# pierregab/VUB_Image_denoising

Measured on AMD Instinct MI355X. Metric: images/sec (256x256x3) RDUNet diffusion train step, higher is better.
Workload: dtype bf16; 1 GPU; RDUNet_T(base_filters=32) diffusion train step, fwd+Charbonnier+bwd+clip+AdamW; global_batch=16, per_gpu_batch=16, parallelism=dp1, optimizer_step=every step, launcher=single process

## Files before the change

vub_image_denoising_amd/csrc/pack.hip:

```cpp
#include "rdn_pointwise.h"

namespace {

__global__ void interp_kernel(const float* __restrict__ clean, const float* __restrict__ noisy,
                              const float* __restrict__ tn, int batch, int64_t per, float* __restrict__ x) {
  const int64_t n4 = per / 4;
  const int64_t total = (int64_t)batch * n4;
  for (int64_t i = (int64_t)blockIdx.x * blockDim.x + threadIdx.x; i < total; i += (int64_t)gridDim.x * blockDim.x) {
    const int b = (int)(i / n4);
    const float a = tn[b];
    const f32x4 c = ((const f32x4*)clean)[i], n = ((const f32x4*)noisy)[i];
    ((f32x4*)x)[i] = a * n + (1.f - a) * c;
  }
}

template <typename T>
__global__ void pack_input_kernel(const float* __restrict__ x, int N, int C, int H, int W, const float* __restrict__ t,
                                  int64_t t_sb, int64_t t_sh, int64_t t_sw, int has_t, T* __restrict__ out, int cpad) {
  const int64_t HW = (int64_t)H * W, P = (int64_t)N * HW;
  for (int64_t p = (int64_t)blockIdx.x * blockDim.x + threadIdx.x; p < P; p += (int64_t)gridDim.x * blockDim.x) {
    const int64_t n = p / HW, r = p - n * HW;
    const int y = (int)(r / W), xx = (int)(r - (int64_t)y * W);
    T* o = out + p * cpad;
    for (int c = 0; c < cpad; ++c) {
      float v = 0.f;
      if (c < C) v = x[(n * C + c) * HW + r];
      else if (c == C && has_t) v = t[n * t_sb + y * t_sh + xx * t_sw];
      o[c] = from_f32<T>(v);
    }
  }
}

__device__ __forceinline__ float pack_value(int mode, const float* __restrict__ w, int d0, int d1, int kh, int kw,
                                            int pad0, int pad1, int kc, int ck, int r, int k) {
  const int taps = kh * kw;
  if (mode == RDN_PACK_CONV_FWD) {
    int tap, b;
    if (ck > 0) { const int ch = k / kc, rem = k - ch * kc; tap = rem / ck; b = ch * ck + (rem - tap * ck); }
    else { tap = k / pad1; b = k - tap * pad1; }
    const int a = r;
    if (a < d0 && b < d1 && tap < taps) return w[((int64_t)a * d1 + b) * taps + tap];
  } else if (mode == RDN_PACK_CONV_DGRAD) {
    int tp, a;
    if (ck > 0) { const int ch = k / kc, rem = k - ch * kc; tp = rem / ck; a = ch * ck + (rem - tp * ck); }
    else { tp = k / pad0; a = k - tp * pad0; }
    const int b = r;
    if (a < d0 && b < d1 && tp < taps) {
      const int ky = kh - 1 - tp / kw, kx = kw - 1 - tp % kw;
      return w[((int64_t)a * d1 + b) * taps + ky * kw + kx];
    }
  } else {
    const int tap = r / d1, b = r - tap * d1, a = k;
    if (tap < taps && a < d0) return w[((int64_t)a * d1 + b) * taps + tap];
  }
  return 0.f;
}

static inline int chunk_sk(int dtype) { return dtype == RDN_BF16 ? 64 : 32; }
static inline int chunk_kc(int ck, int dtype) {
  const int sk = chunk_sk(dtype);
  return ck > 0 ? (9 * ck + sk - 1) / sk * sk : 0;
}

template <typename T>
__global__ void pack_weights_kernel(int mode, const float* __restrict__ w, int d0, int d1, int kh, int kw, int pad0,
                                    int pad1, T* __restrict__ out, int rows_pad, int kp, int ck, int kc) {
  const int64_t total = (int64_t)rows_pad * kp;
  for (int64_t i = (int64_t)blockIdx.x * blockDim.x + threadIdx.x; i < total; i += (int64_t)gridDim.x * blockDim.x) {
    const int r = (int)(i / kp), k = (int)(i - (int64_t)r * kp);
    out[i] = from_f32<T>(pack_value(mode, w, d0, d1, kh, kw, pad0, pad1, kc, ck, r, k));
  }
}

template <typename T>
__global__ __launch_bounds__(256) void pack_weights_batched_kernel(const rdn_pack_item* __restrict__ items, int sk) {
  constexpr int VEC = TypeInfo<T>::VEC;
  const rdn_pack_item it = items[blockIdx.y];
  const int kc = it.ck > 0 ? (9 * it.ck + sk - 1) / sk * sk : 0;
  const int units = it.rows_pad * (it.kp / VEC);
  T* __restrict__ out = (T*)it.out;
  for (int u = blockIdx.x * 256 + threadIdx.x; u < units; u += gridDim.x * 256) {
    const int e = u * VEC, r = e / it.kp, k0 = e - r * it.kp;
    float v[VEC];
#pragma unroll
    for (int q = 0; q < VEC; ++q)
      v[q] = pack_value(it.mode, it.w, it.d0, it.d1, it.kh, it.kw, it.pad0, it.pad1, kc, it.ck, r, k0 + q);
    *(u32x4*)(out + e) = Unit16<T>::pack(v);
  }
}

__global__ void sampling_combine_kernel(float* __restrict__ x, const float* __restrict__ f1, const float* __restrict__ f2,
                                        const float* __restrict__ y, int64_t n, float c1, float a, float c2, float ap) {
#pragma clang fp contract(off)
  for (int64_t i = (int64_t)blockIdx.x * blockDim.x + threadIdx.x; i < n; i += (int64_t)gridDim.x * blockDim.x) {
    const float xt = c1 * f1[i] + a * y[i];
    const float xp = c2 * f2[i] + ap * y[i];
    x[i] = (x[i] - xt) + xp;
  }
}

template <typename T>
__global__ void nchw_to_nhwc_kernel(const float* __restrict__ s, int N, int C, int H, int W, T* __restrict__ d,
                                    int64_t ps, int c0, int64_t pl, int acc) {
  const int64_t HW = (int64_t)H * W, total = (int64_t)N * C * HW;
  for (int64_t i = (int64_t)blockIdx.x * blockDim.x + threadIdx.x; i < total; i += (int64_t)gridDim.x * blockDim.x) {
    const int64_t p = i / C;
    const int c = (int)(i - p * C);
    const int64_t n = p / HW, r = p - n * HW;
    T* const o = d + p * ps + rdn_coff(c0 + c, ps, pl);
    const float v = s[(n * C + c) * HW + r];
    *o = from_f32<T>(acc ? to_f32(*o) + v : v);
  }
}

template <typename T>
__global__ void nhwc_to_nchw_kernel(const T* __restrict__ s, int64_t ps, int c0, int64_t pl, int N, int C, int H, int W,
                                    float* __restrict__ d, int acc) {
  const int64_t HW = (int64_t)H * W, total = (int64_t)N * C * HW;
  for (int64_t i = (int64_t)blockIdx.x * blockDim.x + threadIdx.x; i < total; i += (int64_t)gridDim.x * blockDim.x) {
    const int64_t r = i % HW, nc = i / HW;
    const int c = (int)(nc % C);
    const int64_t n = nc / C;
    const float v = to_f32(s[(n * HW + r) * ps + rdn_coff(c0 + c, ps, pl)]);
    d[i] = acc ? d[i] + v : v;
  }
}

template <typename T>
__global__ void zero_slice_kernel(T* __restrict__ d, int64_t pixels, int64_t ps, int c0, int cols) {
  const int64_t total = pixels * cols;
  for (int64_t i = (int64_t)blockIdx.x * blockDim.x + threadIdx.x; i < total; i += (int64_t)gridDim.x * blockDim.x) {
    const int64_t p = i / cols;
    const int c = (int)(i - p * cols);
    d[p * ps + c0 + c] = from_f32<T>(0.f);
  }
}

}

extern "C" int rdn_interp(const float* clean, const float* noisy, const float* tnorm, int32_t batch, int64_t per,
                          float* x, void* stream) {
  if (!clean || !noisy || !tnorm || !x || per % 4 || ((uintptr_t)clean | (uintptr_t)noisy | (uintptr_t)x) & 15) {
    rdn_set_error("rdn_interp: bad arguments"); return RDN_E_ARG;
  }
  interp_kernel<<<grid_for(batch * per / 4, 256), 256, 0, RDN_STREAM>>>(clean, noisy, tnorm, batch, per, x);
  return rdn_check_launch("rdn_interp");
}

extern "C" int rdn_pack_input(int32_t dtype, const float* x, int32_t n, int32_t c, int32_t h, int32_t w, const float* t,
                              int64_t t_sb, int64_t t_sh, int64_t t_sw, int32_t has_t, void* out, int32_t cpad,
                              void* stream) {
  if (!x || !out || (has_t && !t) || cpad < c + (has_t ? 1 : 0)) { rdn_set_error("rdn_pack_input: bad arguments"); return RDN_E_ARG; }
  const int64_t P = (int64_t)n * h * w;
  RDN_LAUNCH_T(dtype, pack_input_kernel<T><<<grid_for(P, 256), 256, 0, RDN_STREAM>>>(x, n, c, h, w, t, t_sb, t_sh, t_sw, has_t,
                                                                                   (T*)out, cpad));
  return rdn_check_launch("rdn_pack_input");
}

extern "C" int rdn_pack_weights_batched(const rdn_pack_item* items, int32_t n, int32_t dtype, void* stream) {
  if (!items || n <= 0 || n > 65535) { rdn_set_error("rdn_pack_weights_batched: bad arguments"); return RDN_E_ARG; }
  dim3 grid(96, n);
  RDN_LAUNCH_T(dtype, pack_weights_batched_kernel<T><<<grid, 256, 0, RDN_STREAM>>>(items, chunk_sk(dtype)));
  return rdn_check_launch("rdn_pack_weights_batched");
}

extern "C" int rdn_pack_weights(int32_t mode, int32_t dtype, const float* w, int32_t d0, int32_t d1, int32_t kh,
                                int32_t kw, int32_t pad0, int32_t pad1, void* out, int32_t rows_pad, int32_t kp,
                                int32_t ck, void* stream) {
  if (!w || !out || mode < 0 || mode > 2 || kp % 64 || rows_pad % 128) { rdn_set_error("rdn_pack_weights: bad arguments"); return RDN_E_ARG; }
  const int taps = kh * kw;
  const int kc = chunk_kc(ck, dtype);
  if (ck > 0) {
    const int kside = mode == RDN_PACK_CONV_FWD ? pad1 : pad0;
    if (taps != 9 || mode == RDN_PACK_GEMM_T || kside % ck || (kside / ck) * kc > kp) {
      rdn_set_error("rdn_pack_weights: chunked pack needs a 3x3 conv mode and kp >= %d", (kside / ck) * kc);
      return RDN_E_SHAPE;
    }
  } else if ((mode == RDN_PACK_CONV_FWD && (pad1 < d1 || rows_pad < d0 || taps * pad1 > kp)) ||
      (mode == RDN_PACK_CONV_DGRAD && (pad0 < d0 || rows_pad < d1 || taps * pad0 > kp)) ||
      (mode == RDN_PACK_GEMM_T && (pad0 < d0 || pad0 > kp || rows_pad < taps * d1))) {
    rdn_set_error("rdn_pack_weights: shape (mode=%d d0=%d d1=%d pad0=%d pad1=%d rows=%d kp=%d)", mode, d0, d1, pad0, pad1,
                  rows_pad, kp);
    return RDN_E_SHAPE;
  }
  const int64_t total = (int64_t)rows_pad * kp;
  RDN_LAUNCH_T(dtype, pack_weights_kernel<T><<<grid_for(total, 256), 256, 0, RDN_STREAM>>>(mode, w, d0, d1, kh, kw, pad0, pad1,
                                                                                         (T*)out, rows_pad, kp, ck, kc));
  return rdn_check_launch("rdn_pack_weights");
}

extern "C" int rdn_sampling_combine(float* x, const float* f1, const float* f2, const float* y, int64_t count, float c1,
                                    float a, float c2, float ap, void* stream) {
  if (!x || !f1 || !f2 || !y || count <= 0) { rdn_set_error("rdn_sampling_combine: bad arguments"); return RDN_E_ARG; }
  sampling_combine_kernel<<<grid_for(count, 256 * 4), 256, 0, RDN_STREAM>>>(x, f1, f2, y, count, c1, a, c2, ap);
  return rdn_check_launch("rdn_sampling_combine");
}

extern "C" int rdn_nchw_to_nhwc(int32_t dtype, const float* src, int32_t n, int32_t c, int32_t h, int32_t w, void* dst,
                                int64_t dst_ps, int32_t dst_c0, int64_t dst_pl, int32_t accumulate, void* stream) {
  if (!src || !dst || dst_ps <= 0) { rdn_set_error("rdn_nchw_to_nhwc: null / bad stride"); return RDN_E_ARG; }
  const int64_t total = (int64_t)n * c * h * w;
  RDN_LAUNCH_T(dtype, nchw_to_nhwc_kernel<T><<<grid_for(total, 256 * 4), 256, 0, RDN_STREAM>>>(src, n, c, h, w, (T*)dst, dst_ps,
                                                                                             dst_c0, dst_pl, accumulate));
  return rdn_check_launch("rdn_nchw_to_nhwc");
}

extern "C" int rdn_nhwc_to_nchw(int32_t dtype, const void* src, int64_t src_ps, int32_t src_c0, int64_t src_pl, int32_t n,
                                int32_t c, int32_t h, int32_t w, float* dst, int32_t accumulate, void* stream) {
  if (!src || !dst || src_ps <= 0) { rdn_set_error("rdn_nhwc_to_nchw: null / bad stride"); return RDN_E_ARG; }
  const int64_t total = (int64_t)n * c * h * w;
  RDN_LAUNCH_T(dtype, nhwc_to_nchw_kernel<T><<<grid_for(total, 256 * 4), 256, 0, RDN_STREAM>>>((const T*)src, src_ps, src_c0, src_pl,
                                                                                             n, c, h, w, dst, accumulate));
  return rdn_check_launch("rdn_nhwc_to_nchw");
}

extern "C" int rdn_zero_slice(int32_t dtype, void* dst, int64_t pixels, int64_t ps, int32_t c0, int32_t cols, void* stream) {
  if (!dst || pixels < 0 || cols < 0) { rdn_set_error("rdn_zero_slice: bad arguments"); return RDN_E_ARG; }
  if (pixels == 0 || cols == 0) return RDN_OK;
  RDN_LAUNCH_T(dtype, zero_slice_kernel<T><<<grid_for(pixels * cols, 256 * 4), 256, 0, RDN_STREAM>>>((T*)dst, pixels, ps, c0, cols));
  return rdn_check_launch("rdn_zero_slice");
}
```

Measured before the change: 1875 images/s.

## Restructure batched weight pack into LDS-staged tiles with balanced persistent scheduling

```diff
diff --git a/vub_image_denoising_amd/csrc/pack.hip b/vub_image_denoising_amd/csrc/pack.hip
--- a/vub_image_denoising_amd/csrc/pack.hip
+++ b/vub_image_denoising_amd/csrc/pack.hip
@@ -1,3 +1,5 @@
+#include "rdn_device.h"
+#include "rdn_launch.h"
 #include "rdn_pointwise.h"
 
 namespace {
@@ -72,20 +74,224 @@
   }
 }
 
-template <typename T>
-__global__ __launch_bounds__(256) void pack_weights_batched_kernel(const rdn_pack_item* __restrict__ items, int sk) {
+constexpr int PK_XT = 64;
+constexpr int PK_RT = 8;
+constexpr int PK_NT = 256;
+constexpr int PK_U = 5;
+constexpr int PK_SLOTS = PK_NT * PK_U;
+constexpr int PK_LDS = PK_XT * 82;
+constexpr int PK_IPT = 2;
+constexpr int PK_MAXN = PK_NT * PK_IPT;
+
+__device__ __forceinline__ int div_small(int i, float inv) { return (int)(((float)i + 0.5f) * inv); }
+
+struct PackGeom {
+  int taps, kc, seg_w, chunk_k, pitch, rt, row_span, taps_out, nch, nxt, ntiles;
+  bool fwd, gemm, gather;
+};
+
+template <typename T>
+__device__ __forceinline__ PackGeom pack_geom(const rdn_pack_item& it, int sk) {
   constexpr int VEC = TypeInfo<T>::VEC;
-  const rdn_pack_item it = items[blockIdx.y];
-  const int kc = it.ck > 0 ? (9 * it.ck + sk - 1) / sk * sk : 0;
-  const int units = it.rows_pad * (it.kp / VEC);
+  PackGeom g;
+  g.taps = it.kh * it.kw;
+  g.kc = it.ck > 0 ? (9 * it.ck + sk - 1) / sk * sk : 0;
+  g.fwd = it.mode == RDN_PACK_CONV_FWD, g.gemm = it.mode == RDN_PACK_GEMM_T;
+  g.seg_w = g.gemm ? it.kp : it.ck > 0 ? it.ck : g.fwd ? it.pad1 : it.pad0;
+  g.chunk_k = it.ck > 0 ? g.kc : it.kp;
+  const int taps1 = max(g.taps, 1);
+  g.rt = g.fwd ? min(PK_RT, PK_SLOTS / ((PK_XT * taps1 + 6) / 4)) : min(32, (4 * (PK_SLOTS / PK_XT) - 3) / taps1);
+  g.pitch = g.fwd ? PK_XT * taps1 + 1 : (g.rt * taps1 + 6) / 8 * 8 + 1;
+  g.gather = g.taps <= 0 || g.seg_w <= 0 || g.seg_w % VEC || it.d0 <= 0 || it.d1 <= 0 || g.chunk_k <= 0 ||
+             it.rows_pad >= (1 << 20) ||
+             (it.ck > 0 && g.taps * g.seg_w > g.chunk_k) || g.rt <= 0 || (g.fwd ? g.rt : PK_XT) * g.pitch > PK_LDS;
+  if (g.gather) {
+    g.ntiles = (it.rows_pad * (it.kp / VEC) + PK_NT - 1) / PK_NT;
+    return g;
+  }
+  g.row_span = g.gemm ? it.d1 : it.rows_pad;
+  g.taps_out = g.gemm ? (it.rows_pad + it.d1 - 1) / it.d1 : g.taps;
+  g.nch = (it.kp + g.chunk_k - 1) / g.chunk_k, g.nxt = (g.seg_w + PK_XT - 1) / PK_XT;
+  g.ntiles = (g.row_span + g.rt - 1) / g.rt * g.nch * g.nxt;
+  return g;
+}
+
+template <typename T>
+__device__ void pack_gather_box(const rdn_pack_item& it, const PackGeom& g, int tile) {
+  constexpr int VEC = TypeInfo<T>::VEC;
+  const int u = tile * PK_NT + threadIdx.x;
+  if (u >= it.rows_pad * (it.kp / VEC)) return;
+  const int e = u * VEC, r = e / it.kp, k0 = e - r * it.kp;
+  float v[VEC];
+#pragma unroll
+  for (int q = 0; q < VEC; ++q)
+    v[q] = pack_value(it.mode, it.w, it.d0, it.d1, it.kh, it.kw, it.pad0, it.pad1, g.kc, it.ck, r, k0 + q);
+  *(u32x4*)((T*)it.out + e) = Unit16<T>::pack(v);
+}
+
+struct PackBox {
+  int xt, ch, r0, xw, xbase, rows_l;
+};
+__device__ __forceinline__ PackBox pack_box_at(const PackGeom& g, int tile) {
+  PackBox b;
+  b.xt = tile % g.nxt, b.ch = (tile / g.nxt) % g.nch, b.r0 = (tile / (g.nxt * g.nch)) * g.rt;
+  b.xw = min(PK_XT, g.seg_w - b.xt * PK_XT);
+  b.xbase = (g.gemm ? 0 : b.ch * g.seg_w) + b.xt * PK_XT;
+  b.rows_l = min(g.rt, g.row_span - b.r0);
+  return b;
+}
+
+struct PackRegs {
+  f32x4 f[PK_U];
+  int l0[PK_U], lo[PK_U], hi[PK_U];
+};
+
+__device__ __forceinline__ void pack_box_fetch(const rdn_pack_item& it, const PackGeom& g, int tile, PackRegs& R) {
+  const PackBox b = pack_box_at(g, tile);
+  const int taps = g.taps, total = it.d0 * it.d1 * taps;
+  const int wal = (int)(((uintptr_t)it.w >> 2) & 3);
+  const float* __restrict__ wa = it.w - wal;
+  const int a_base = g.fwd ? b.r0 : b.xbase, b_base = g.fwd ? b.xbase : b.r0;
+  const int nruns = max(min(g.fwd ? b.rows_l : b.xw, it.d0 - a_base), 0);
+  const int n = max(min(g.fwd ? b.xw : b.rows_l, it.d1 - b_base), 0) * taps;
+  const int nv = (n + 6) / 4;
+  const float inv_nv = 1.f / (float)nv;
+#pragma unroll
+  for (int s = 0; s < PK_U; ++s) {
+    const int i = threadIdx.x + s * PK_NT;
+    R.lo[s] = R.hi[s] = R.l0[s] = 0;
+    if (n == 0 || i >= nruns * nv) continue;
+    const int j = div_small(i, inv_nv), v = i - j * nv;
+    const int g0 = wal + ((a_base + j) * it.d1 + b_base) * taps;
+    const int e0 = (g0 & ~3) + 4 * v;
+    R.l0[s] = j * g.pitch + e0 - g0;
+    R.lo[s] = max(g0 - e0, 0), R.hi[s] = min(g0 + n - e0, 4);
+    if (e0 >= wal && e0 + 4 <= wal + total) R.f[s] = *(const f32x4*)(wa + e0);
+    else {
+#pragma unroll
+      for (int q = 0; q < 4; ++q)
+        if (q >= R.lo[s] && q < R.hi[s]) R.f[s][q] = wa[e0 + q];
+    }
+  }
+}
+
+__device__ __forceinline__ void pack_box_stage(const PackRegs& R, float* __restrict__ lds) {
+#pragma unroll
+  for (int s = 0; s < PK_U; ++s) {
+    if (R.lo[s] == 0 && R.hi[s] == 4) {
+#pragma unroll
+      for (int q = 0; q < 4; ++q) lds[R.l0[s] + q] = R.f[s][q];
+    } else {
+#pragma unroll
+      for (int q = 0; q < 4; ++q)
+        if (q >= R.lo[s] && q < R.hi[s]) lds[R.l0[s] + q] = R.f[s][q];
+    }
+  }
+}
+
+template <typename T>
+__device__ __forceinline__ void pack_box_emit(const rdn_pack_item& it, const PackGeom& g, int tile,
+                                              const float* __restrict__ lds) {
+  constexpr int VEC = TypeInfo<T>::VEC, XG = PK_XT / VEC;
+  const PackBox b = pack_box_at(g, tile);
+  const bool fwd = g.fwd, gemm = g.gemm;
+  const int taps = g.taps, seg_w = g.seg_w;
   T* __restrict__ out = (T*)it.out;
-  for (int u = blockIdx.x * 256 + threadIdx.x; u < units; u += gridDim.x * 256) {
-    const int e = u * VEC, r = e / it.kp, k0 = e - r * it.kp;
+  const int sr = fwd ? g.pitch : taps, sx = fwd ? taps : g.pitch;
+  const int xg_n = b.xw / VEC;
+  const int k_box = b.ch * g.chunk_k + b.xt * PK_XT;
+  const int xlim = (fwd ? it.d1 : it.d0) - b.xbase, rlim = (fwd ? it.d0 : it.d1) - b.r0;
+  const float inv_to = 1.f / (float)g.taps_out;
+  for (int u = threadIdx.x; u < b.rows_l * g.taps_out * XG; u += PK_NT) {
+    const int xg = u % XG, rest = u / XG, r_l = div_small(rest, inv_to), t = rest - r_l * g.taps_out;
+    const int k = k_box + (gemm ? 0 : t * seg_w) + xg * VEC;
+    const int row = b.r0 + r_l + (gemm ? t * it.d1 : 0);
+    if (xg >= xg_n || k >= it.kp || row >= it.rows_pad) continue;
+    const int nok = (r_l < rlim && t < taps) ? xlim - xg * VEC : 0;
+    const float* const l = lds + r_l * sr + xg * VEC * sx + (it.mode == RDN_PACK_CONV_DGRAD ? taps - 1 - t : t);
     float v[VEC];
-#pragma unroll
-    for (int q = 0; q < VEC; ++q)
-      v[q] = pack_value(it.mode, it.w, it.d0, it.d1, it.kh, it.kw, it.pad0, it.pad1, kc, it.ck, r, k0 + q);
-    *(u32x4*)(out + e) = Unit16<T>::pack(v);
+    if (nok >= VEC) {
+#pragma unroll
+      for (int q = 0; q < VEC; ++q) v[q] = l[q * sx];
+    } else {
+#pragma unroll
+      for (int q = 0; q < VEC; ++q) v[q] = q < nok ? l[q * sx] : 0.f;
+    }
+    *(u32x4*)(out + row * it.kp + k) = Unit16<T>::pack(v);
+  }
+  const int tail0 = b.ch * g.chunk_k + taps * seg_w, tail1 = min((b.ch + 1) * g.chunk_k, it.kp);
+  if (!gemm && b.xt == g.nxt - 1 && tail0 < tail1) {
+    const int tu = (tail1 - tail0) / VEC;
+    for (int u = threadIdx.x; u < b.rows_l * tu; u += PK_NT) {
+      const int r_l = u / tu, k = tail0 + (u - r_l * tu) * VEC;
+      *(u32x4*)(out + (b.r0 + r_l) * it.kp + k) = u32x4{0u, 0u, 0u, 0u};
+    }
+  }
+}
+
+template <typename T>
+__global__ __launch_bounds__(PK_NT) void pack_weights_batched_kernel(const rdn_pack_item* __restrict__ items, int n,
+                                                                      int sk) {
+  __shared__ float lds[PK_LDS];
+  __shared__ int pre[PK_MAXN + 1];
+  __shared__ int wsum[PK_NT / 64];
+  int c[PK_IPT], s = 0;
+#pragma unroll
+  for (int q = 0; q < PK_IPT; ++q) {
+    const int i = threadIdx.x * PK_IPT + q;
+    c[q] = i < n ? pack_geom<T>(items[i], sk).ntiles : 0;
+    s += c[q];
+  }
+  const int lane = threadIdx.x & 63, wv = threadIdx.x >> 6;
+  int incl = s;
+#pragma unroll
+  for (int o = 1; o < 64; o <<= 1) {
+    const int up = __shfl_up(incl, o, 64);
+    if (lane >= o) incl += up;
+  }
+  if (lane == 63) wsum[wv] = incl;
+  __syncthreads();
+  int run = incl - s;
+  for (int w = 0; w < wv; ++w) run += wsum[w];
+  if (threadIdx.x == 0) pre[0] = 0;
+#pragma unroll
+  for (int q = 0; q < PK_IPT; ++q) {
+    run += c[q];
+    pre[threadIdx.x * PK_IPT + q + 1] = run;
+  }
+  __syncthreads();
+  const int total = __builtin_amdgcn_readfirstlane(pre[n]), per = (total + gridDim.x - 1) / gridDim.x;
+  const int t0 = blockIdx.x * per, t1 = min(total, t0 + per);
+  if (t0 >= t1) return;
+  int lo = 0, hi = n - 1;
+  while (lo < hi) {
+    const int mid = (lo + hi + 1) >> 1;
+    if (__builtin_amdgcn_readfirstlane(pre[mid]) <= t0) lo = mid; else hi = mid - 1;
+  }
+  auto locate = [&](int tile, int& i, rdn_pack_item& it, PackGeom& g) {
+    const int was = i;
+    while (__builtin_amdgcn_readfirstlane(pre[i + 1]) <= tile) ++i;
+    if (i != was || tile == t0) { it = items[i]; g = pack_geom<T>(it, sk); }
+    return tile - __builtin_amdgcn_readfirstlane(pre[i]);
+  };
+  rdn_pack_item it, it_n;
+  PackGeom g, g_n;
+  PackRegs R;
+  int box = locate(t0, lo, it, g);
+  if (!g.gather) pack_box_fetch(it, g, box, R);
+  for (int tile = t0; tile < t1; ++tile) {
+    if (!g.gather) pack_box_stage(R, lds);
+    bar_lds();
+    int box_n = 0;
+    it_n = it, g_n = g;
+    if (tile + 1 < t1) {
+      box_n = locate(tile + 1, lo, it_n, g_n);
+      if (!g_n.gather) pack_box_fetch(it_n, g_n, box_n, R);
+    }
+    if (g.gather) pack_gather_box<T>(it, g, box);
+    else pack_box_emit<T>(it, g, box, lds);
+    bar_lds();
+    it = it_n, g = g_n, box = box_n;
   }
 }
 
@@ -157,10 +363,18 @@
   return rdn_check_launch("rdn_pack_input");
 }
 
+template <typename T>
+static int pack_grid() {
+  static const int g = rdn_cu_count() * resident_per_cu(pack_weights_batched_kernel<T>, PK_NT, 8);
+  return g;
+}
+
 extern "C" int rdn_pack_weights_batched(const rdn_pack_item* items, int32_t n, int32_t dtype, void* stream) {
   if (!items || n <= 0 || n > 65535) { rdn_set_error("rdn_pack_weights_batched: bad arguments"); return RDN_E_ARG; }
-  dim3 grid(96, n);
-  RDN_LAUNCH_T(dtype, pack_weights_batched_kernel<T><<<grid, 256, 0, RDN_STREAM>>>(items, chunk_sk(dtype)));
+  for (int i = 0; i < n; i += PK_MAXN) {
+    const int m = n - i < PK_MAXN ? n - i : PK_MAXN;
+    RDN_LAUNCH_T(dtype, pack_weights_batched_kernel<T><<<pack_grid<T>(), PK_NT, 0, RDN_STREAM>>>(items + i, m, chunk_sk(dtype)));
+  }
   return rdn_check_launch("rdn_pack_weights_batched");
 }
 
```

Result: no change. 1881 images/s, median of 6 (+0.3%).
